# RozDavid/UnScene3D

Measured on AMD Instinct MI355X. Metric: training scenes/sec (Res16UNet34C+Mask3D, 150k voxels), higher is better.
Workload: dtype f32

## Files before the change

### include/usc3d.h

```cpp
#ifndef USC3D_H
#define USC3D_H

#include <stdint.h>

#ifdef __cplusplus
extern "C" {
#endif

typedef void* usc_stream_t;

enum usc_status {
  USC_OK = 0,
  USC_ERR_ARG = -1,
  USC_ERR_LAUNCH = -2,
  USC_ERR_RANGE = -3
};

const char* usc_last_error(void);
int usc_abi_version(void);
const char* usc_build_info(void);
int usc_device_count(void);


int usc_voxel_floor_f64(const double* xyz, int64_t n, double voxel_size,
// ... 550 lines not shown
int usc_adamw_step(float* param, const float* grad, float* exp_avg, float* exp_avg_sq,
                   int64_t n, float lr, float beta1, float beta2, float eps,
                   float weight_decay, int64_t step, usc_stream_t s);

int usc_adamw_step_scaled(float* param, float* grad, float* exp_avg, float* exp_avg_sq, int64_t n,
                          float grad_scale, int32_t write_back_grad,
                          float lr, float beta1, float beta2, float eps, float weight_decay,
                          int64_t step, usc_stream_t s);

int usc_elastic_displace(const void* xyz_in, int32_t is_f64, int64_t n, int32_t row_stride,
                         const float* noise, int32_t dim_x, int32_t dim_y, int32_t dim_z,
                         const double* axis_x, const double* axis_y, const double* axis_z,
                         double magnitude, void* xyz_out, usc_stream_t s);

int usc_affine_rows(void* x, int32_t is_f64, int64_t n, int32_t row_stride,
                    const double* M, const double* t, usc_stream_t s);
int usc_colsum_sequential(const float* x, int64_t n, int32_t row_stride,
                          int32_t cols, float* out, usc_stream_t s);
int usc_color_lut(const float* color, int64_t n, int32_t row_stride,
                  const float* lut, float* out, int32_t out_stride,
                  usc_stream_t s);

int usc_felz_face_normals(const float* vertices, const int32_t* faces,
                          int64_t n_faces, float* face_normals, usc_stream_t s);
int usc_felz_vertex_normals(const float* face_normals, const int64_t* corner_order,
                            const int64_t* vertex_off, int64_t n_vertices,
                            float* normals, usc_stream_t s);
int usc_felz_edge_weights(const float* vertices, const float* colors,
                          const float* normals, const int32_t* faces,
                          int64_t n_faces, int32_t* edge_a, int32_t* edge_b,
                          float* weights, usc_stream_t s);
int usc_felz_merge_host(const int32_t* edge_a, const int32_t* edge_b,
                        const float* weights, int64_t n_edges, int32_t n_vertices,
                        float kthr, int32_t seg_min_verts, int32_t* comps);

int usc_mask_gt_overlap(const uint8_t* masks, int64_t n, int32_t k, int64_t ld,
                        const int32_t* slot, int32_t nslots, int32_t* counts,
                        usc_stream_t s);

int32_t usc_vit_attn_head_dim(void);
int usc_vit_attn_fwd(const float* qkv, int32_t B, int32_t T, int32_t H, float scale,
                     int32_t precision, float* o, usc_stream_t s);

int usc_instance_index(const int64_t* labels, int64_t n, int32_t ld, const int64_t* ids, int32_t u,
                       int32_t* rank, int32_t* count, int32_t* first, usc_stream_t s);
int usc_instance_select(const int64_t* labels, int64_t n, int32_t ld, const int64_t* ids, int32_t u,
                        const int32_t* count, const int32_t* first, const int64_t* filter, int32_t nf,
                        int64_t label_offset, int32_t* slot, int64_t* labels_out, int32_t* n_kept,
                        usc_stream_t s);
int usc_instance_masks(const int32_t* rank, int64_t n, const int32_t* slot, int32_t u, int32_t t,
                       uint8_t* masks, const int64_t* seg, int32_t seg_ld, int64_t n_segments,
                       uint8_t* segment_mask, usc_stream_t s);

int usc_freemask_normalize(const float* feats, int64_t n, int32_t c, float* scale, uint8_t* zero, usc_stream_t s);
int64_t usc_freemask_ws_bytes(int64_t q, int64_t k);
int usc_freemask_rowstats(const float* fq, const float* sq, int64_t q, const float* fk, const float* sk, int64_t k,
                          int32_t c, float* rowmin, float* rowmax, void* ws, int64_t ws_bytes, usc_stream_t s);
int usc_freemask_bits(const float* fq, const float* sq, int64_t q, const float* fk, const float* sk,
                      const uint8_t* zero_k, int64_t k, int32_t c, const float* rowmin, const float* rowmax,
                      float threshold, uint64_t* bits, int32_t* count, float* soft_sum, void* ws, int64_t ws_bytes,
                      usc_stream_t s);
int usc_freemask_soft_rows(const float* fq, const float* sq, int64_t q, const float* fk, const float* sk,
                           const uint8_t* zero_k, int64_t k, int32_t c, const float* rowmin, const float* rowmax,
                           const int32_t* qidx, int32_t m, float* out, usc_stream_t s);
int usc_mask_bits_extent(const uint64_t* bits, int64_t n, int64_t k, const int32_t* coords, int32_t* lo, int32_t* hi,
                         usc_stream_t s);
int64_t usc_mask_bits_nms_ws_bytes(int64_t n);
int usc_mask_bits_nms(const uint64_t* bits, const int32_t* count, int64_t k, const int32_t* order, int32_t n,
                      float nms_thr, uint8_t* keep, void* ws, int64_t ws_bytes, usc_stream_t s);

#define USC_MASK_BITS_MAX_SEGMENTS 8192
int32_t usc_mask_bits_max_segments(void);
int usc_maxpool_down2_i32(const int32_t* in, int64_t n_fine, const int32_t* nbr2, int64_t n_coarse, int32_t* out,
                          usc_stream_t s);
int usc_mask_bits_components(const uint64_t* bits, int64_t n_bits_rows, int32_t n_segments, const int32_t* rows,
                             int32_t n_rows, const int64_t* adj_off, const int32_t* adj, int32_t* label,
                             int32_t* n_comp, usc_stream_t s);
int usc_mask_bits_split(const int32_t* label, int32_t n_rows, int32_t n_segments, const int64_t* row_off,
                        const int32_t* n_comp, const int32_t* weight, const float* soft, int64_t soft_ld,
                        const int32_t* soft_row, uint64_t* out_bits, int32_t* out_src, int32_t* out_root,
                        int32_t* seg_count, int32_t* vox_count, float* soft_sum, usc_stream_t s);
int usc_mask_bits_nms_weighted(const uint64_t* bits, const int32_t* count, const int32_t* weight, int64_t k,
                               const int32_t* order, int32_t n, float nms_thr, uint8_t* keep, void* ws,
                               int64_t ws_bytes, usc_stream_t s);

int64_t usc_softmask_stats_ws_bytes(int64_t n, int32_t k);
int usc_softmask_stats(const float* soft, const float* xyz, int64_t n, int32_t k, float thr, int32_t* count, float* lo,
                       float* hi, void* ws, int64_t ws_bytes, usc_stream_t s);
int usc_softmask_table(const float* soft, int64_t n, int32_t k, float thr, const int32_t* keep, int32_t kk,
                       const float* segments, int32_t* out, usc_stream_t s);
int usc_mesh_vertex_normals(const float* vertices, const int32_t* faces, const int64_t* corner_order,
                            const int64_t* vertex_off, int64_t n_vertices, int64_t n_faces, float* normals,
                            usc_stream_t s);

int usc_mask_columns_to_bits(const uint8_t* masks, int64_t n, int32_t k, uint64_t* bits, int32_t* count,
                             usc_stream_t s);
int usc_mask_bits_gather(const uint64_t* src, int64_t m, const int64_t* ind, int64_t n, int32_t k, uint64_t* dst,
                         int32_t* count, usc_stream_t s);
int usc_mask_bits_count(const uint64_t* bits, int32_t k, int64_t n, int32_t* count, usc_stream_t s);
int32_t usc_selftrain_merge_lds_words(int32_t words);
int usc_selftrain_merge(const uint64_t* st, const int32_t* total, int32_t kp, int64_t n, uint64_t* fg,
                        int32_t max_add, uint64_t* fresh, int32_t* picked, int32_t* n_added, usc_stream_t s);
int usc_mask_bits_to_columns(const uint64_t* bits, const int32_t* rows, int32_t m, int64_t n, float* out, int64_t ld,
                             int32_t col0, usc_stream_t s);
int usc_mask_bits_to_columns_u8(const uint64_t* bits, const int32_t* rows, int32_t m, int64_t n, uint8_t* out,
                                int64_t ld, int32_t col0, usc_stream_t s);
// ... 17 lines not shown
```

### unscene3d_amd/_lib.py

```python
from __future__ import annotations

import ctypes as C
import os

import torch

_HERE = os.path.dirname(os.path.abspath(__file__))
LIB_PATH = os.environ.get("USC3D_LIB") or os.path.join(_HERE, "libusc3d_hip.so")

_p = C.c_void_p
_i32 = C.c_int32
_i64 = C.c_int64
_f64 = C.c_double
_f32 = C.c_float

class KMap(C.Structure):
    _fields_ = [("nbr", _p), ("perm", _p), ("tile_mask", _p), ("pair_in", _p), ("pair_out", _p), ("koff", _p),
                ("n_in", _i64), ("n_out", _i64), ("pair_capacity", _i64), ("K", _i32), ("reserved", _i32)]


class BNDesc(C.Structure):
    _fields_ = [("gamma", _p), ("beta", _p), ("running_mean", _p), ("running_var", _p), ("num_batches_tracked", _p),
                ("eps", _f32), ("momentum", _f32), ("c", _i32), ("training", _i32)]

# ... 152 lines not shown
    "usc_adamw_step_scaled": (C.c_int, [_p, _p, _p, _p, _i64, _f32, _i32, _f32, _f32, _f32, _f32, _f32, _i64, _p]),
    "usc_elastic_displace": (C.c_int, [_p, _i32, _i64, _i32, _p, _i32, _i32, _i32, _p, _p, _p, _f64, _p, _p]),
    "usc_attn_max_queries": (_i32, []),
    "usc_attn_lse_stride": (_i32, [_i32]),
    "usc_attn_ws_bytes": (_i64, [_i32, _i32, _i32, _i32]),
    "usc_attn_fwd": (C.c_int, [_p, _p, _p, _p, _i32, _i32, _i32, _i32, _i32, _p, _p, _p, _i64, _p]),
    "usc_attn_bwd": (C.c_int, [_p, _p, _p, _p, _p, _p, _p, _i32, _i32, _i32, _i32, _i32, _p, _p, _p, _i32, _p, _i64, _p]),
    "usc_lsap_batch": (C.c_int, [_p, _i32, _i32, _i32, _p, _p, _p, _p]),
    "usc_criterion_ws_bytes": (_i64, [_i32, _i32, _i32]),
    "usc_criterion_ws_bytes_q": (_i64, [_i32, _i32, _i32, _i32]),
    "usc_criterion_target_bits": (C.c_int, [_p, _i32, _i32, _i32, _p, _p, _p]),
    "usc_criterion_costs": (C.c_int, [_p, _i32, _i32, _i32, _i32, _i32, _i32, _p, _p, _p, _i64, _i64, _i32, _p, _f32, _f32,
                                      _f32, _p, _p, _p, _p, _p, _p, _p, _i64, _p]),
    "usc_criterion_drop_counts": (C.c_int, [_p, _i32, _i32, _i32, _i32, _i32, _i32, _p, _p, _p, _p, _p]),
    "usc_criterion_losses": (C.c_int, [_p, _p, _p, _p, _p, _p, _p, _i32, _i32, _i32, _i32, _i32, _i32, _p, _p, _p, _p,
                                       _f32, _p, _p]),
    "usc_criterion_table": (C.c_int, [_p, _i32, _i32, _p, _p, _p]),
    "usc_criterion_backward": (C.c_int, [_p, _p, _i32, _i32, _i32, _i32, _i32, _i32, _p, _p, _p, _p, _p, _p, _p, _p, _p,
                                         _p, _p, _i32, _i64, _i64, _p, _p, _p]),
    "usc_self_attn_fwd": (C.c_int, [_p, _p, _p, _i32, _i32, _i32, _i32, _p, _p, _p]),
    "usc_self_attn_bwd": (C.c_int, [_p, _p, _p, _p, _p, _p, _i32, _i32, _i32, _i32, _p, _p, _p, _p]),
    "usc_linear_fwd": (C.c_int, [_p, _p, _p, _i32, _i32, _i32, _p, _p]),
    "usc_linear_bwd": (C.c_int, [_p, _p, _p, _i32, _i32, _i32, _p, _p, _p, _i32, _p]),
    "usc_layernorm_fwd": (C.c_int, [_p, _p, _p, _i64, _i32, _f32, _p, _p, _p, _p]),
    "usc_add_layernorm_fwd": (C.c_int, [_p, _p, _p, _p, _i64, _i32, _f32, _p, _p, _p, _p, _p]),
    "usc_linear_fwd_ex": (C.c_int, [_p, _p, _p, _p, _i32, _i32, _i32, _i32, _p, _p]),
    "usc_linear_fwd_pad": (C.c_int, [_p, _p, _p, _p, _i32, _i32, _i32, _i32, _p, _i32, _p]),
    "usc_linear_fwd_split": (C.c_int, [_p, _p, _p, _p, _i32, _i32, _i32, _i32, _i32, _p, _p]),
    "usc_linear_bwd_ex": (C.c_int, [_p, _p, _p, _p, _p, _i32, _i32, _i32, _p, _p, _p, _p, _i32, _p]),
    "usc_qkv_proj_bwd": (C.c_int, [_p, _p, _p, _p, _i32, _i32, _p, _p, _p, _p, _p, _i32, _p]),
    "usc_linear_bwd_ex2": (C.c_int, [_p, _p, _p, _p, _p, _i32, _i32, _i32, _p, _p, _p, _p, _p, _p, _i32, _p]),
    "usc_linear_heads_max": (_i32, []),
    "usc_linear_heads_dx": (C.c_int, [_p, _p, _i32, _i32, _i32, _i32, _p, _p]),
    "usc_layernorm_bwd_ws_bytes": (_i64, [_i64, _i32]),
    "usc_layernorm_bwd": (C.c_int, [_p, _p, _p, _p, _p, _i64, _i32, _p, _p, _p, _i32, _p, _i64, _p]),
    "usc_layernorm_bwd_ex": (C.c_int, [_p, _p, _p, _p, _p, _i64, _i32, _p, _p, _p, _p, _i32, _p, _i64, _p]),
    "usc_affine_rows": (C.c_int, [_p, _i32, _i64, _i32, _p, _p, _p]),
    "usc_colsum_sequential": (C.c_int, [_p, _i64, _i32, _i32, _p, _p]),
    "usc_col_sum_ws_bytes": (_i64, [_i64, _i32]),
    "usc_col_sum": (C.c_int, [_p, _i64, _i32, _p, _i32, _p, _i64, _p]),
    "usc_color_lut": (C.c_int, [_p, _i64, _i32, _p, _p, _i32, _p]),
    "usc_felz_face_normals": (C.c_int, [_p, _p, _i64, _p, _p]),
    "usc_felz_vertex_normals": (C.c_int, [_p, _p, _p, _i64, _p, _p]),
    "usc_felz_edge_weights": (C.c_int, [_p, _p, _p, _p, _i64, _p, _p, _p, _p]),
    "usc_felz_merge_host": (C.c_int, [_p, _p, _p, _i64, _i32, _f32, _i32, _p]),
    "usc_furthest_point_sampling": (C.c_int, [_p, _i32, _i32, _i32, _p, _p, _p]),
    "usc_fourier_posenc": (C.c_int, [_p, _i64, _p, _p, _p, _i32, _p, _p]),
    "usc_mask_gt_overlap": (C.c_int, [_p, _i64, _i32, _i64, _p, _i32, _p, _p]),
    "usc_vit_attn_head_dim": (_i32, []),
    "usc_vit_attn_fwd": (C.c_int, [_p, _i32, _i32, _i32, _f32, _i32, _p, _p]),
    "usc_instance_index": (C.c_int, [_p, _i64, _i32, _p, _i32, _p, _p, _p, _p]),
    "usc_instance_select": (C.c_int, [_p, _i64, _i32, _p, _i32, _p, _p, _p, _i32, _i64, _p, _p, _p, _p]),
    "usc_instance_masks": (C.c_int, [_p, _i64, _p, _i32, _i32, _p, _p, _i32, _i64, _p, _p]),
    "usc_freemask_normalize": (C.c_int, [_p, _i64, _i32, _p, _p, _p]),
    "usc_freemask_ws_bytes": (_i64, [_i64, _i64]),
    "usc_freemask_rowstats": (C.c_int, [_p, _p, _i64, _p, _p, _i64, _i32, _p, _p, _p, _i64, _p]),
    "usc_freemask_bits": (C.c_int, [_p, _p, _i64, _p, _p, _p, _i64, _i32, _p, _p, _f32, _p, _p, _p, _p, _i64, _p]),
    "usc_freemask_soft_rows": (C.c_int, [_p, _p, _i64, _p, _p, _p, _i64, _i32, _p, _p, _p, _i32, _p, _p]),
    "usc_mask_bits_extent": (C.c_int, [_p, _i64, _i64, _p, _p, _p, _p]),
    "usc_mask_bits_nms_ws_bytes": (_i64, [_i64]),
    "usc_mask_bits_nms": (C.c_int, [_p, _p, _i64, _p, _i32, _f32, _p, _p, _i64, _p]),
    "usc_mask_bits_max_segments": (_i32, []),
    "usc_maxpool_down2_i32": (C.c_int, [_p, _i64, _p, _i64, _p, _p]),
    "usc_mask_bits_components": (C.c_int, [_p, _i64, _i32, _p, _i32, _p, _p, _p, _p, _p]),
    "usc_mask_bits_split": (C.c_int, [_p, _i32, _i32, _p, _p, _p, _p, _i64, _p, _p, _p, _p, _p, _p, _p, _p]),
    "usc_mask_bits_nms_weighted": (C.c_int, [_p, _p, _p, _i64, _p, _i32, _f32, _p, _p, _i64, _p]),
    "usc_softmask_stats_ws_bytes": (_i64, [_i64, _i32]),
    "usc_softmask_stats": (C.c_int, [_p, _p, _i64, _i32, _f32, _p, _p, _p, _p, _i64, _p]),
    "usc_softmask_table": (C.c_int, [_p, _i64, _i32, _f32, _p, _i32, _p, _p, _p]),
    "usc_mesh_vertex_normals": (C.c_int, [_p, _p, _p, _p, _i64, _i64, _p, _p]),
    "usc_mask_columns_to_bits": (C.c_int, [_p, _i64, _i32, _p, _p, _p]),
    "usc_mask_bits_gather": (C.c_int, [_p, _i64, _p, _i64, _i32, _p, _p, _p]),
    "usc_mask_bits_count": (C.c_int, [_p, _i32, _i64, _p, _p]),
    "usc_selftrain_merge_lds_words": (_i32, [_i32]),
    "usc_selftrain_merge": (C.c_int, [_p, _p, _i32, _i64, _p, _i32, _p, _p, _p, _p]),
    "usc_mask_bits_to_columns": (C.c_int, [_p, _p, _i32, _i64, _p, _i64, _i32, _p]),
    "usc_mask_bits_to_columns_u8": (C.c_int, [_p, _p, _i32, _i64, _p, _i64, _i32, _p]),
    "usc_mask_bits_max_segments_wide": (_i32, []),
    "usc_mask_columns_to_segment_bits": (C.c_int, [_p, _i64, _i32, _p, _p, _i32, _p, _p]),
    "usc_mask_bits_components_wide": (C.c_int, [_p, _i64, _i32, _p, _i32, _p, _p, _p, _p, _p, _p]),
    "usc_segment_parts_to_columns": (C.c_int, [_p, _i32, _i32, _p, _p, _i32, _p, _i64, _p, _p]),
}


class LaunchStat(C.Structure):
    _fields_ = [("n_out", _i64), ("cin", _i32), ("cout", _i32), ("K", _i32), ("nb", _i32)]


def _load():
    if not os.path.exists(LIB_PATH):
        raise ImportError(
            f"{LIB_PATH} is missing: build the HIP extension first "
            "(`python -c 'import __graft_entry__ as g; g.build()'`). "
            "unscene3d_amd has no CPU fallback."
        )
    lib = C.CDLL(LIB_PATH)
    for name, (res, args) in SIGNATURES.items():
        fn = getattr(lib, name)
        fn.restype = res
        fn.argtypes = args
    return lib


lib = _load()
if lib.usc_step_size() != C.sizeof(Step):
    raise ImportError(f"unscene3d_amd._lib.Step ({C.sizeof(Step)} bytes) does not mirror usc_step "
# ... 19 lines not shown
```

### unscene3d_amd/csrc/targets.hip

```cpp
#include "common.h"

namespace usc {

constexpr int kTgtBlock = 256;
constexpr int kTgtWindow = 2048;
constexpr int kTgtWaveRows = 256;
constexpr int kTgtRowsPerBlock = 8;

__global__ void instance_index_init_kernel(int32_t u, int32_t* __restrict__ count, int32_t* __restrict__ first) {
  for (int32_t i = blockIdx.x * blockDim.x + threadIdx.x; i < u; i += gridDim.x * blockDim.x) {
    count[i] = 0;
    first[i] = INT32_MAX;
  }
}

__device__ inline int32_t find_rank(const int64_t* __restrict__ ids, int32_t u, int64_t v) {
  int32_t lo = 0, hi = u;
  while (lo < hi) {
    const int32_t mid = (lo + hi) >> 1;
    if (ids[mid] < v) lo = mid + 1; else hi = mid;
  }
  return (lo < u && ids[lo] == v) ? lo : -1;
}

// ... 87 lines not shown
  const int64_t base = ((int64_t)blockIdx.x * (kTgtBlock / 64) + wave) * kTgtWaveRows;
  if (base >= n) return;
  const int len = (int)min((int64_t)kTgtWaveRows, n - base);

  int32_t sl[4];
#pragma unroll
  for (int k = 0; k < 4; ++k) {
    const int64_t r = base + 64 * k + lane;
    sl[k] = -1;
    if (r < n) {
      const int32_t q = rank[r];
      if ((uint32_t)q < (uint32_t)u) {
        const int32_t t = slot[q];
        if ((uint32_t)t < (uint32_t)t_total) sl[k] = t;
      }
    }
  }
  if (segment_mask != nullptr && blockIdx.y == 0) {
#pragma unroll
    for (int k = 0; k < 4; ++k) {
      if (sl[k] >= 0) {
        const int64_t sg = seg[(base + 64 * k + lane) * seg_ld];
        if ((uint64_t)sg < (uint64_t)s) segment_mask[(int64_t)sl[k] * s + sg] = 1;
      }
    }
  }

  const int t0 = blockIdx.y * kTgtRowsPerBlock;
  const int t1 = min(t_total, t0 + kTgtRowsPerBlock);
  for (int t = t0; t < t1; ++t) {
    const uint64_t b0 = __ballot(sl[0] == t), b1 = __ballot(sl[1] == t);
    const uint64_t b2 = __ballot(sl[2] == t), b3 = __ballot(sl[3] == t);
    uint8_t* row = masks + (int64_t)t * n + base;
    const int m = (int)((uintptr_t)row & 3);
    const int j_lo = m ? 1 : 0;
    const int j_hi = (len + m) >> 2;
    if (lane >= j_lo && lane < j_hi) {
      const int i0 = 4 * lane - m;
      const int q = i0 >> 6, o = i0 & 63;
      const uint64_t cur = q == 0 ? b0 : q == 1 ? b1 : q == 2 ? b2 : b3;
      const uint64_t nxt = q == 0 ? b1 : q == 1 ? b2 : q == 2 ? b3 : 0;
      uint32_t bits = (uint32_t)(cur >> o);
      if (o > 60) bits |= (uint32_t)(nxt << (64 - o));
      const uint32_t word = (bits & 1u) | ((bits & 2u) << 7) | ((bits & 4u) << 14) | ((bits & 8u) << 21);
      *reinterpret_cast<uint32_t*>(row + i0) = word;
    }
    const int head_n = min(max(4 * j_lo - m, 0), len);
    if (lane < head_n) row[lane] = (uint8_t)ballot_bit(b0, b1, b2, b3, lane);
    const int tail = max(4 * j_hi - m, head_n) + lane;
    if (tail < len) row[tail] = (uint8_t)ballot_bit(b0, b1, b2, b3, tail);
  }
}

}

using namespace usc;

extern "C" {

int usc_instance_index(const int64_t* labels, int64_t n, int32_t ld, const int64_t* ids, int32_t u, int32_t* rank,
                       int32_t* count, int32_t* first, usc_stream_t s) {
  USC_REQUIRE(n >= 0 && n < INT32_MAX, "usc_instance_index: n out of range [0, 2^31-2]");
  USC_REQUIRE(ld >= 2, "usc_instance_index: ld < 2 (the instance id is column 1)");
  USC_REQUIRE(u >= 0 && u <= 65535 * kTgtWindow, "usc_instance_index: u out of range");
  USC_REQUIRE(u == 0 || (ids && count && first), "usc_instance_index: null pointer");
  USC_REQUIRE(n == 0 || (labels && rank), "usc_instance_index: null pointer");
  USC_REQUIRE(n == 0 || u > 0, "usc_instance_index: rows without ids");
  hipStream_t st = as_stream(s);
  if (u == 0) return USC_OK;
  hipLaunchKernelGGL(instance_index_init_kernel, dim3(stream_grid(u, kTgtBlock)), dim3(kTgtBlock), 0, st, u, count,
                     first);
  USC_CHECK_LAUNCH("usc_instance_index");
  if (n == 0) return USC_OK;
  const dim3 grid(stream_grid(n, kTgtBlock), (unsigned)ceil_div(u, kTgtWindow));
  hipLaunchKernelGGL(instance_index_kernel, grid, dim3(kTgtBlock), 0, st, labels, n, ld, ids, u, rank, count, first);
  USC_CHECK_LAUNCH("usc_instance_index");
  return USC_OK;
}

int usc_instance_select(const int64_t* labels, int64_t n, int32_t ld, const int64_t* ids, int32_t u,
                        const int32_t* count, const int32_t* first, const int64_t* filter, int32_t nf,
                        int64_t label_offset, int32_t* slot, int64_t* labels_out, int32_t* n_kept, usc_stream_t s) {
  USC_REQUIRE(n >= 0 && n < INT32_MAX, "usc_instance_select: n out of range [0, 2^31-2]");
  USC_REQUIRE(ld >= 1, "usc_instance_select: ld < 1");
  USC_REQUIRE(u >= 0, "usc_instance_select: u < 0");
  USC_REQUIRE(nf >= 0 && (nf == 0 || filter), "usc_instance_select: bad filter list");
  USC_REQUIRE(n_kept, "usc_instance_select: null n_kept");
  USC_REQUIRE(u == 0 || (labels && ids && count && first && slot && labels_out), "usc_instance_select: null pointer");
  hipLaunchKernelGGL(instance_select_kernel, dim3(1), dim3(kTgtBlock), 0, as_stream(s), labels, ld, ids, u, count,
                     first, filter, nf, label_offset, slot, labels_out, n_kept);
  USC_CHECK_LAUNCH("usc_instance_select");
  return USC_OK;
}

int usc_instance_masks(const int32_t* rank, int64_t n, const int32_t* slot, int32_t u, int32_t t, uint8_t* masks,
                       const int64_t* seg, int32_t seg_ld, int64_t n_segments, uint8_t* segment_mask,
                       usc_stream_t s) {
  USC_REQUIRE(n >= 0 && n < INT32_MAX, "usc_instance_masks: n out of range [0, 2^31-2]");
  USC_REQUIRE(u >= 0, "usc_instance_masks: u < 0");
  USC_REQUIRE(t >= 0 && t <= u && t <= 65535 * kTgtRowsPerBlock, "usc_instance_masks: t out of range [0, u]");
  USC_REQUIRE(n_segments >= 0, "usc_instance_masks: n_segments < 0");
  if (t == 0 || n == 0) return USC_OK;
  USC_REQUIRE(rank && slot && masks, "usc_instance_masks: null pointer");
  if (n_segments == 0) segment_mask = nullptr;
  USC_REQUIRE(segment_mask == nullptr || (seg && seg_ld >= 1), "usc_instance_masks: segment_mask without segment ids");
  const dim3 grid((unsigned)ceil_div(n, (kTgtBlock / 64) * kTgtWaveRows), (unsigned)ceil_div(t, kTgtRowsPerBlock));
  hipLaunchKernelGGL(instance_masks_kernel, grid, dim3(kTgtBlock), 0, as_stream(s), rank, n, slot, u, t, masks, seg,
                     seg_ld, n_segments, segment_mask);
  USC_CHECK_LAUNCH("usc_instance_masks");
  return USC_OK;
}
// ... 3 lines not shown
```

### unscene3d_amd/datasets/utils.py

```python
from __future__ import annotations

import numpy as np
import torch

from .. import MinkowskiEngine as ME
from .. import ops


def _dev(x, dev, dtype):
    t = x if isinstance(x, torch.Tensor) else torch.as_tensor(np.asarray(x))
    return t.to(device=dev, dtype=dtype).contiguous()


class NoGpu:

    def __init__(self, coordinates, features, original_labels=None, inverse_maps=None, full_res_coords=None,
                 target_full=None, original_colors=None, original_normals=None, original_coordinates=None, idx=None,
                 segment_connectivity=None):
        self.coordinates, self.features = coordinates, features
        self.original_labels, self.inverse_maps, self.full_res_coords = original_labels, inverse_maps, full_res_coords
        self.target_full, self.original_colors, self.original_normals = target_full, original_colors, original_normals
        self.original_coordinates, self.idx, self.segment_connectivity = original_coordinates, idx, segment_connectivity


def get_instance_freemasks(list_freemasks, list_segments=None):
    target = []
    for b, table in enumerate(list_freemasks):
        colsT = (table[:, 1:-1] != 0).T.contiguous()
        keep = torch.nonzero(colsT.any(1)).reshape(-1)
        if keep.numel() == 0:
            return []
        masks = colsT[keep]
        entry = {"labels": torch.ones(keep.numel(), dtype=torch.int64, device=table.device), "masks": masks}
        if list_segments:
            S = list_segments[b].shape[0]
            tt, rr = torch.nonzero(masks, as_tuple=True)
            vals = table[rr]
            sm = torch.zeros((keep.numel(), S), dtype=torch.bool, device=table.device)
            sm[tt[:, None].expand_as(vals).reshape(-1), vals.reshape(-1)] = True
            entry["segment_mask"] = sm
        target.append(entry)
    return target


def freemask_voxelize(batch, ignore_label, voxel_size, mode, ignore_class_threshold, device="cuda",
                      spatial_sort=False):
    dev = torch.device(device)
    coords_l, feats_l, tables, inverse_maps = [], [], [], []
    full_res_coords, original_freemasks, colors, normals, raw_coords, idx, seg_conn = [], [], [], [], [], [], []
    for sample in batch:
        full_res_coords.append(sample[0])
        original_freemasks.append(sample[2])
        colors.append(sample[4])
        normals.append(sample[5])
        raw_coords.append(sample[6])
        idx.append(sample[7])
        seg_conn.append(sample[8])
        xyz = _dev(sample[0], dev, torch.float64)
        c3, unique_map, inverse_map = ME.utils.sparse_quantize(xyz, quantization_size=voxel_size, return_index=True,
                                                               return_inverse=True, device=str(dev))
        if spatial_sort:
            c4 = torch.cat([torch.zeros((c3.shape[0], 1), dtype=torch.int32, device=dev), c3], 1).contiguous()
            order = ops.spatial_order(c4, shift=int(spatial_sort) if spatial_sort is not True else 3)
            rank = torch.empty_like(order)
            rank[order] = torch.arange(order.shape[0], device=dev)
            c3, unique_map, inverse_map = c3[order], unique_map[order], rank[inverse_map]
        inverse_maps.append(inverse_map)
        coords_l.append(c3.int())
        feats_l.append(_dev(sample[1], dev, torch.float32)[unique_map])
        if len(sample[2]) > 0:
            tables.append(_dev(sample[2], dev, torch.int64)[unique_map])

    if tables:
        width = max(t.shape[1] for t in tables)
        tables = [torch.cat([t[:, :-1], t.new_zeros(t.shape[0], width - t.shape[1]), t[:, -1:]], dim=1) for t in tables]
        coordinates, features, _ = ME.utils.sparse_collate(coords_l, feats_l, tables)
    else:
        coordinates, features = ME.utils.sparse_collate(coords_l, feats_l)

    target, target_full = [], []
    if tables:
        segment2label, n_segments = [], []
        for t in tables:
            seg = t[:, -1]
            uniq, inv = torch.unique(seg, return_inverse=True)
            n_segments.append(int(uniq.shape[0]))
            first = torch.full((uniq.shape[0],), seg.shape[0], dtype=torch.long, device=dev)
            first.scatter_reduce_(0, inv, torch.arange(seg.shape[0], device=dev), reduce="amin")
            t[:, -1] = inv
            segment2label.append(t[first][:, :-1])
        target = get_instance_freemasks(tables, list_segments=segment2label)
        for i in range(len(target)):
            target[i]["point2segment"] = tables[i][:, -1].contiguous()
            target[i]["num_segments"] = torch.tensor(n_segments[i])
        full = [m if isinstance(m, torch.Tensor) else torch.as_tensor(np.asarray(m)) for m in original_freemasks]
        target_full = get_instance_freemasks(full)
        for i in range(len(target_full)):
            target_full[i]["point2segment"] = full[i][:, -1].long()
    else:
        coordinates, features = [], []
    return (NoGpu(coordinates, features, original_freemasks, inverse_maps, full_res_coords, target_full, colors,
                  normals, raw_coords, idx, seg_conn), target, [sample[3] for sample in batch])


class FreeMaskVoxelizeCollate:
    def __init__(self, ignore_label=255, voxel_size=1, mode="test", small_crops=False, very_small_crops=False,
                 batch_instance=False, probing=False, task="instance_segmentation", ignore_class_threshold=100,
                 filter_out_classes=(), label_offset=0, num_queries=None, device="cuda", spatial_sort=False):
        assert task in ["instance_segmentation"], "task not known"
        if small_crops or very_small_crops:
            raise NotImplementedError("crop collates are outside the accelerated path (SURVEY.md §2.1)")
        self.ignore_label, self.voxel_size, self.mode = ignore_label, voxel_size, mode
        self.ignore_class_threshold, self.device, self.spatial_sort = ignore_class_threshold, device, spatial_sort

    def __call__(self, batch):
        return freemask_voxelize(batch, self.ignore_label, self.voxel_size, self.mode, self.ignore_class_threshold,
                                 device=self.device, spatial_sort=self.spatial_sort)


def get_instance_masks(list_labels, task, list_segments=None, ignore_class_threshold=100, filter_out_classes=(),
                       label_offset=0):
    if task == "semantic_segmentation":
        raise NotImplementedError("task='semantic_segmentation' targets are outside the accelerated path (SURVEY.md §2.1)")
    target = []
# ... 116 lines not shown
```

### unscene3d_amd/ops.py

```python
from __future__ import annotations

from dataclasses import dataclass

import ctypes
import os
import weakref

import torch

from . import profiler as _prof
from ._lib import check, lib, require_device


def _stream():
    return torch._C._cuda_getCurrentRawStream(torch._C._cuda_getDevice())


def _chk(t: torch.Tensor, dtype, name: str):
    if not isinstance(t, torch.Tensor):
        raise RuntimeError(f"{name} must be a torch.Tensor")
    if not t.is_cuda:
        raise RuntimeError(f"{name} must be a HIP (cuda) tensor — unscene3d_amd has no CPU path")
    if t.dtype != dtype:
        raise RuntimeError(f"{name} must be {dtype}, got {t.dtype}")
# ... 983 lines not shown
                            _ptr(d2), _ptr(ws), ws.numel(), _stream()), "usc_knn1_grid")
    return d2.sqrt(), idx


def mask_gt_overlap(masks: torch.Tensor, slot: torch.Tensor, nslots: int) -> torch.Tensor:
    require_device()
    if not isinstance(masks, torch.Tensor) or masks.dim() != 2 or not masks.is_cuda:
        raise RuntimeError("masks must be a 2-D HIP (cuda) tensor")
    if masks.dtype == torch.bool:
        masks = masks.view(torch.uint8)
    if masks.dtype != torch.uint8:
        raise RuntimeError(f"masks must be bool or uint8, got {masks.dtype}")
    n, k = masks.shape
    if n > 0 and (masks.stride(1) != 1 or masks.stride(0) < k):
        masks = masks.contiguous()
    ld = masks.stride(0) if n > 0 else k
    _chk(slot, torch.int32, "slot")
    if slot.shape != (n,):
        raise RuntimeError(f"slot must be [{n}], got {list(slot.shape)}")
    counts = torch.empty((k + 1, int(nslots)), dtype=torch.int32, device=masks.device)
    check(lib.usc_mask_gt_overlap(_ptr(masks), n, k, ld, _ptr(slot), int(nslots), _ptr(counts), _stream()),
          "usc_mask_gt_overlap")
    return counts


def instance_targets(labels: torch.Tensor, num_segments=None, filter_out_classes=(), label_offset: int = 0, alloc=None):
    require_device()
    _chk(labels, torch.int64, "labels")
    if labels.dim() != 2 or labels.shape[1] < (2 if num_segments is None else 3):
        raise RuntimeError("labels must be [N, >= 2] (with segments: [N, >= 3])")
    dev = labels.device
    if alloc is None:
        def alloc(shape, dtype, zero):
            return (torch.zeros if zero else torch.empty)(shape, dtype=dtype, device=dev)
    n, ld = labels.shape
    ids = torch.unique(labels[:, 1]).contiguous()
    u = int(ids.shape[0])
    rank, count, first = alloc((n,), torch.int32, False), alloc((u,), torch.int32, False), alloc((u,), torch.int32, False)
    slot, lab, kept = alloc((u,), torch.int32, False), alloc((u,), torch.int64, False), alloc((1,), torch.int32, False)
    flt = torch.tensor([int(c) for c in filter_out_classes], dtype=torch.int64, device=dev)
    st = _stream()
    check(lib.usc_instance_index(_ptr(labels), n, ld, _ptr(ids), u, _ptr(rank), _ptr(count), _ptr(first), st),
          "usc_instance_index")
    check(lib.usc_instance_select(_ptr(labels), n, ld, _ptr(ids), u, _ptr(count), _ptr(first), _ptr(flt),
                                  int(flt.shape[0]), int(label_offset), _ptr(slot), _ptr(lab), _ptr(kept), st),
          "usc_instance_select")
    t = int(kept.item())
    masks = alloc((t, n), torch.uint8, False)
    seg_mask = None if num_segments is None else alloc((t, int(num_segments)), torch.uint8, True)
    check(lib.usc_instance_masks(_ptr(rank), n, _ptr(slot), u, t, _ptr(masks), _ptr(labels[:, 2:]) if seg_mask is not None
                                 else None, ld, 0 if seg_mask is None else int(num_segments), _ptr(seg_mask), st),
          "usc_instance_masks")
    return lab[:t], masks.view(torch.bool), None if seg_mask is None else seg_mask.view(torch.bool)


VIT_ATTN_PRECISIONS = {"f32": 0, "bf16": 1}


def vit_attention(qkv: torch.Tensor, B: int, T: int, H: int, scale: float, precision: str = "f32") -> torch.Tensor:
    require_device()
    _chk(qkv, torch.float32, "qkv")
    if precision not in VIT_ATTN_PRECISIONS:
        raise RuntimeError(f"precision must be 'f32' or 'bf16', got {precision!r}")
    d = lib.usc_vit_attn_head_dim()
    if qkv.numel() != B * T * 3 * H * d:
        raise RuntimeError(f"qkv must hold [B={B}, T={T}, 3, H={H}, {d}] values, got {list(qkv.shape)}")
    o = torch.empty((B, T, H * d), dtype=torch.float32, device=qkv.device)
    check(lib.usc_vit_attn_fwd(_ptr(qkv), B, T, H, float(scale), VIT_ATTN_PRECISIONS[precision], _ptr(o), _stream()),
          "usc_vit_attn_fwd")
    return o


def cc_eps(xyz: torch.Tensor, eps: float, max_rounds: int = 256) -> torch.Tensor:
    require_device()
    _chk(xyz, torch.float32, "xyz")
    n = xyz.shape[0]
    dev = xyz.device
    la = torch.empty(n, dtype=torch.int32, device=dev)
    lb = torch.empty(n, dtype=torch.int32, device=dev)
    changed = torch.zeros(1, dtype=torch.int32, device=dev)
    check(lib.usc_cc_eps_init(_ptr(la), n, _stream()), "usc_cc_eps_init")
    for _ in range(max_rounds):
        check(lib.usc_cc_eps_step(_ptr(xyz), n, float(eps), _ptr(la), _ptr(lb), _ptr(changed), _stream()),
              "usc_cc_eps_step")
        la, lb = lb, la
        if int(changed.item()) == 0:
            break
    else:
        raise RuntimeError("cc_eps: label propagation did not converge")
    labels = torch.empty(n, dtype=torch.int64, device=dev)
    check(lib.usc_cc_eps_finish(_ptr(la), n, _ptr(lb), _ptr(labels), _stream()), "usc_cc_eps_finish")
    return labels


DBSCAN_OFF = -2
DBSCAN_MAX_CELLS_PER_AXIS = 1 << 20


def dbscan_masks(xyz: torch.Tensor, masks: torch.Tensor, eps: float, min_samples: int = 1):
    require_device()
    _chk(xyz, torch.float32, "xyz")
    _chk(masks, torch.float32, "masks")
    if xyz.dim() != 2 or xyz.shape[1] != 3 or masks.dim() != 2 or masks.shape[0] != xyz.shape[0]:
        raise RuntimeError(f"dbscan_masks: xyz must be [N,3] and masks [N,Q], got {list(xyz.shape)}, {list(masks.shape)}")
    eps32 = ctypes.c_float(float(eps)).value
    if not (eps32 > 0.0) or eps32 == float("inf"):
# ... 740 lines not shown
```

Before: 46.84.

## Build freemask training targets natively with hash-based segment indexing on GPU

Adds native HIP kernels that scan the per-scene label table once, find which mask columns are non-empty, build a hash table of segment ids, rank them, and emit masks, point2segment and segment masks directly. This replaces the torch-op path (gather, unique, pad, scatter_reduce, per-target mask building) in freemask_voxelize and is enabled by default through an environment flag. The new path needs one pinned-memory readback per table to learn the target and segment counts. The rank kernel is quadratic in the number of segments and the collate path now skips the padded-table concatenation.

```diff
diff --git a/include/usc3d.h b/include/usc3d.h
--- a/include/usc3d.h
+++ b/include/usc3d.h
@@ -626,6 +626,17 @@
                        uint8_t* masks, const int64_t* seg, int32_t seg_ld, int64_t n_segments,
                        uint8_t* segment_mask, usc_stream_t s);
 
+int64_t usc_freemask_targets_ws_bytes(int64_t n, int32_t W, int32_t with_segments);
+int usc_freemask_targets_index(const void* src, int32_t src_i64, int32_t W, const int64_t* rows,
+                               int64_t n_src, int64_t n, int32_t with_segments, void* ws,
+                               int64_t ws_bytes, int64_t* out_table, int32_t Wp, int64_t* host_counts,
+                               usc_stream_t s);
+int usc_freemask_targets_emit(const void* src, int32_t src_i64, int32_t W, const int64_t* rows,
+                              int64_t n_src, int64_t n, int32_t with_segments, void* ws,
+                              int64_t ws_bytes, int32_t T, int64_t S, uint8_t* masks, int64_t* labels,
+                              int64_t* point2segment, uint8_t* segment_mask, int64_t* out_table,
+                              int32_t Wp, int64_t* segment2label, usc_stream_t s);
+
 int usc_freemask_normalize(const float* feats, int64_t n, int32_t c, float* scale, uint8_t* zero, usc_stream_t s);
 int64_t usc_freemask_ws_bytes(int64_t q, int64_t k);
 int usc_freemask_rowstats(const float* fq, const float* sq, int64_t q, const float* fk, const float* sk, int64_t k,
diff --git a/unscene3d_amd/_lib.py b/unscene3d_amd/_lib.py
--- a/unscene3d_amd/_lib.py
+++ b/unscene3d_amd/_lib.py
@@ -228,6 +228,10 @@
     "usc_instance_index": (C.c_int, [_p, _i64, _i32, _p, _i32, _p, _p, _p, _p]),
     "usc_instance_select": (C.c_int, [_p, _i64, _i32, _p, _i32, _p, _p, _p, _i32, _i64, _p, _p, _p, _p]),
     "usc_instance_masks": (C.c_int, [_p, _i64, _p, _i32, _i32, _p, _p, _i32, _i64, _p, _p]),
+    "usc_freemask_targets_ws_bytes": (_i64, [_i64, _i32, _i32]),
+    "usc_freemask_targets_index": (C.c_int, [_p, _i32, _i32, _p, _i64, _i64, _i32, _p, _i64, _p, _i32, _p, _p]),
+    "usc_freemask_targets_emit": (C.c_int, [_p, _i32, _i32, _p, _i64, _i64, _i32, _p, _i64, _i32, _i64, _p, _p, _p, _p,
+                                            _p, _i32, _p, _p]),
     "usc_freemask_normalize": (C.c_int, [_p, _i64, _i32, _p, _p, _p]),
     "usc_freemask_ws_bytes": (_i64, [_i64, _i64]),
     "usc_freemask_rowstats": (C.c_int, [_p, _p, _i64, _p, _p, _i64, _i32, _p, _p, _p, _i64, _p]),
diff --git a/unscene3d_amd/csrc/targets.hip b/unscene3d_amd/csrc/targets.hip
--- a/unscene3d_amd/csrc/targets.hip
+++ b/unscene3d_amd/csrc/targets.hip
@@ -163,11 +163,344 @@
   }
 }
 
+constexpr int kFmBlock = 256;
+constexpr int kFmMaxCols = 1024;
+constexpr int kFmTile = 1024;
+constexpr int64_t kFmEmpty = INT64_MIN;
+
+struct FmWs {
+  int64_t* counts;
+  int32_t* colflag;
+  int32_t* col_of_t;
+  int64_t* hkeys;
+  int32_t* hidx;
+  int64_t* distinct;
+  int32_t* rslot;
+  int32_t* rank;
+  int32_t* first;
+  int64_t cap, bytes;
+};
+
+static int64_t fm_cap(int64_t n) {
+  int64_t cap = 1024;
+  while (cap < 2 * n) cap <<= 1;
+  return cap;
+}
+
+static FmWs fm_carve(void* ws, int64_t n, int32_t K, bool with_seg) {
+  FmWs w{};
+  char* p = (char*)ws;
+  int64_t o = 0;
+  auto take = [&](int64_t bytes) { char* q = p + o; o += align_up(bytes, 16); return q; };
+  w.counts = (int64_t*)take(32);
+  w.colflag = (int32_t*)take((int64_t)K * 4);
+  w.col_of_t = (int32_t*)take((int64_t)K * 4);
+  if (with_seg) {
+    w.cap = fm_cap(n);
+    w.hkeys = (int64_t*)take(w.cap * 8);
+    w.hidx = (int32_t*)take(w.cap * 4);
+    w.distinct = (int64_t*)take(n * 8);
+    w.rslot = (int32_t*)take(n * 4);
+    w.rank = (int32_t*)take(n * 4);
+    w.first = (int32_t*)take(n * 4);
+  }
+  w.bytes = o;
+  return w;
+}
+
+__global__ void fm_init_kernel(int64_t* __restrict__ counts, int32_t* __restrict__ colflag, int32_t K,
+                               int64_t* __restrict__ hkeys, int64_t cap) {
+  const int64_t i0 = (int64_t)blockIdx.x * blockDim.x + threadIdx.x;
+  if (i0 < 4) counts[i0] = 0;
+  if (i0 < K) colflag[i0] = 0;
+  for (int64_t i = i0; i < cap; i += (int64_t)gridDim.x * blockDim.x) hkeys[i] = kFmEmpty;
+}
+
+template <typename TS>
+__global__ __launch_bounds__(kFmBlock) void fm_scan_kernel(const TS* __restrict__ src, int32_t W,
+                                                           const int64_t* __restrict__ rows, int64_t n_src, int64_t n,
+                                                           int64_t* __restrict__ hkeys, int32_t* __restrict__ hidx,
+                                                           int64_t cap, int64_t* __restrict__ distinct,
+                                                           int32_t* __restrict__ rslot, int32_t* __restrict__ colflag,
+                                                           int64_t* __restrict__ counts, int64_t* __restrict__ out_table,
+                                                           int32_t Wp) {
+  __shared__ int32_t sflag[kFmMaxCols];
+  const int K = W - 2;
+  for (int i = threadIdx.x; i < K; i += kFmBlock) sflag[i] = 0;
+  __syncthreads();
+  for (int64_t r = (int64_t)blockIdx.x * kFmBlock + threadIdx.x; r < n; r += (int64_t)gridDim.x * kFmBlock) {
+    const int64_t q = rows ? rows[r] : r;
+    if ((uint64_t)q >= (uint64_t)n_src) {
+      counts[2] = 1;
+      if (rslot) rslot[r] = -1;
+      continue;
+    }
+    const TS* __restrict__ p = src + q * W;
+    for (int c = 0; c < K; ++c)
+      if (p[1 + c] != 0 && !sflag[c]) sflag[c] = 1;
+    const int64_t sg = (int64_t)p[W - 1];
+    if (rslot) {
+      int32_t mine = -1;
+      if (sg == kFmEmpty) {
+        counts[2] = 1;
+      } else {
+        uint64_t slot = hash_key((uint64_t)sg) & (uint64_t)(cap - 1);
+        for (;;) {
+          if (__atomic_load_n(&hkeys[slot], __ATOMIC_RELAXED) == sg) break;
+          const unsigned long long prev = atomicCAS((unsigned long long*)&hkeys[slot], (unsigned long long)kFmEmpty,
+                                                    (unsigned long long)sg);
+          if (prev == (unsigned long long)kFmEmpty) {
+            const int64_t di = (int64_t)atomicAdd((unsigned long long*)&counts[1], 1ull);
+            distinct[di] = sg;
+            hidx[slot] = (int32_t)di;
+            break;
+          }
+          if (prev == (unsigned long long)sg) break;
+          slot = (slot + 1) & (uint64_t)(cap - 1);
+        }
+        mine = (int32_t)slot;
+      }
+      rslot[r] = mine;
+    }
+    if (out_table) {
+      int64_t* __restrict__ o = out_table + r * Wp;
+      for (int c = 0; c < W - 1; ++c) o[c] = (int64_t)p[c];
+      for (int c = W - 1; c < Wp - 1; ++c) o[c] = 0;
+      o[Wp - 1] = sg;
+    }
+  }
+  __syncthreads();
+  for (int i = threadIdx.x; i < K; i += kFmBlock)
+    if (sflag[i]) colflag[i] = 1;
+}
+
+__global__ void fm_count_kernel(const int32_t* __restrict__ colflag, int32_t K, int32_t* __restrict__ col_of_t,
+                                int64_t* __restrict__ counts) {
+  if (threadIdx.x != 0 || blockIdx.x != 0) return;
+  int32_t t = 0;
+  for (int32_t c = 0; c < K; ++c)
+    if (colflag[c]) col_of_t[t++] = c;
+  counts[0] = t;
+}
+
+__global__ __launch_bounds__(kFmBlock) void fm_rank_kernel(const int64_t* __restrict__ distinct, int64_t S,
+                                                           int32_t* __restrict__ rank, int32_t* __restrict__ first,
+                                                           int64_t* __restrict__ labels, int32_t T) {
+  __shared__ int64_t tile[kFmTile];
+  const int64_t i = (int64_t)blockIdx.x * kFmBlock + threadIdx.x;
+  const int64_t v = i < S ? distinct[i] : 0;
+  int32_t below = 0;
+  for (int64_t j0 = 0; j0 < S; j0 += kFmTile) {
+    const int m = (int)min((int64_t)kFmTile, S - j0);
+    __syncthreads();
+    for (int k = threadIdx.x; k < m; k += kFmBlock) tile[k] = distinct[j0 + k];
+    __syncthreads();
+    for (int k = 0; k < m; ++k) below += tile[k] < v ? 1 : 0;
+  }
+  if (i < S) {
+    rank[i] = below;
+    first[i] = INT32_MAX;
+  }
+  if (i < T) labels[i] = 1;
+}
+
+__device__ inline void fm_mark(uint8_t* __restrict__ row, int64_t S, int64_t v) {
+  if (v < 0) v += S;
+  if ((uint64_t)v < (uint64_t)S) row[v] = 1;
+}
+
+template <typename TS>
+__global__ __launch_bounds__(kFmBlock) void fm_rows_kernel(const TS* __restrict__ src, int32_t W,
+                                                           const int64_t* __restrict__ rows, int64_t n_src, int64_t n,
+                                                           int32_t Wp, int32_t T, int64_t S,
+                                                           const int32_t* __restrict__ col_of_t,
+                                                           const int32_t* __restrict__ rslot,
+                                                           const int32_t* __restrict__ hidx,
+                                                           const int32_t* __restrict__ rank, int32_t* __restrict__ first,
+                                                           int32_t want_first, uint8_t* __restrict__ masks,
+                                                           int64_t* __restrict__ p2s, uint8_t* __restrict__ segmask,
+                                                           int64_t* __restrict__ out_table) {
+  __shared__ int32_t scol[kFmMaxCols];
+  for (int i = threadIdx.x; i < T; i += kFmBlock) scol[i] = col_of_t[i];
+  __syncthreads();
+  const int lane = threadIdx.x & 63;
+  const int K = W - 2;
+  for (int64_t base = (int64_t)blockIdx.x * kFmBlock; base < n; base += (int64_t)gridDim.x * kFmBlock) {
+    const int64_t r = base + threadIdx.x;
+    bool valid = r < n;
+    int64_t q = 0;
+    if (valid) {
+      q = rows ? rows[r] : r;
+      if ((uint64_t)q >= (uint64_t)n_src) { valid = false; q = 0; }
+    }
+    const TS* __restrict__ p = src + q * W;
+    int64_t rk = -1;
+    if (valid && rslot) {
+      const int32_t slot = rslot[r];
+      if (slot >= 0) {
+        rk = rank[hidx[slot]];
+        p2s[r] = rk;
+        if (out_table) out_table[r * Wp + Wp - 1] = rk;
+        if (want_first && rk < S) atomicMin(&first[rk], (int32_t)r);
+      }
+    }
+    bool has0 = false, has1 = false, odd = false;
+    int64_t lab = 0;
+    if (valid && segmask) {
+      lab = (int64_t)p[0];
+      has0 = Wp > W || lab == 0 || rk == 0;
+      has1 = lab == 1 || rk == 1;
+      for (int c = 0; c < K; ++c) {
+        const int64_t v = (int64_t)p[1 + c];
+        has0 = has0 || v == 0;
+        has1 = has1 || v == 1;
+        odd = odd || (v != 0 && v != 1);
+      }
+    }
+    for (int t = 0; t < T; ++t) {
+      const bool bit = valid && p[1 + scol[t]] != 0;
+      if (r < n) masks[(int64_t)t * n + r] = bit ? 1 : 0;
+      if (segmask) {
+        uint8_t* __restrict__ row = segmask + (int64_t)t * S;
+        const uint64_t b0 = __ballot(bit && has0), b1 = __ballot(bit && has1);
+        if (b0 && S > 0 && lane == __ffsll((unsigned long long)b0) - 1) row[0] = 1;
+        if (b1 && S > 1 && lane == __ffsll((unsigned long long)b1) - 1) row[1] = 1;
+        if (bit) {
+          if (rk > 1 && rk < S) row[rk] = 1;
+          if (lab != 0 && lab != 1) fm_mark(row, S, lab);
+          if (odd)
+            for (int c = 0; c < K; ++c) {
+              const int64_t v = (int64_t)p[1 + c];
+              if (v != 0 && v != 1) fm_mark(row, S, v);
+            }
+        }
+      }
+    }
+  }
+}
+
+template <typename TS>
+__global__ void fm_seg2label_kernel(const TS* __restrict__ src, int32_t W, const int64_t* __restrict__ rows,
+                                    int64_t n_src, int64_t n, int32_t Wp, int64_t S,
+                                    const int32_t* __restrict__ first, int64_t* __restrict__ out) {
+  const int64_t total = S * (Wp - 1);
+  for (int64_t e = (int64_t)blockIdx.x * blockDim.x + threadIdx.x; e < total; e += (int64_t)gridDim.x * blockDim.x) {
+    const int64_t sgm = e / (Wp - 1);
+    const int c = (int)(e - sgm * (Wp - 1));
+    const int64_t fr = first[sgm];
+    const int64_t q = fr >= n ? -1 : rows ? rows[fr] : fr;
+    out[e] = (c < W - 1 && (uint64_t)q < (uint64_t)n_src) ? (int64_t)src[q * W + c] : 0;
+  }
+}
+
+static thread_local int64_t* g_fm_pinned = nullptr;
+
 }
 
 using namespace usc;
 
 extern "C" {
+
+int64_t usc_freemask_targets_ws_bytes(int64_t n, int32_t W, int32_t with_segments) {
+  if (n < 0 || W < 2) return 0;
+  return fm_carve(nullptr, n, W - 2, with_segments != 0).bytes;
+}
+
+int usc_freemask_targets_index(const void* src, int32_t src_i64, int32_t W, const int64_t* rows, int64_t n_src,
+                               int64_t n, int32_t with_segments, void* ws, int64_t ws_bytes, int64_t* out_table,
+                               int32_t Wp, int64_t* host_counts, usc_stream_t s) {
+  USC_REQUIRE(n >= 0 && n < INT32_MAX && n_src >= 0, "usc_freemask_targets_index: n out of range [0, 2^31-2]");
+  USC_REQUIRE(W >= 2 && W - 2 <= kFmMaxCols, "usc_freemask_targets_index: table width %d outside [2, %d]", W,
+              kFmMaxCols + 2);
+  USC_REQUIRE(Wp >= W, "usc_freemask_targets_index: padded width below the table's");
+  USC_REQUIRE(ws && host_counts, "usc_freemask_targets_index: null pointer");
+  USC_REQUIRE(n == 0 || src, "usc_freemask_targets_index: null table");
+  USC_REQUIRE(ws_bytes >= usc_freemask_targets_ws_bytes(n, W, with_segments),
+              "usc_freemask_targets_index: workspace too small");
+  USC_REQUIRE(out_table == nullptr || with_segments, "usc_freemask_targets_index: the gathered table needs segments");
+  hipStream_t st = as_stream(s);
+  const int32_t K = W - 2;
+  const FmWs w = fm_carve(ws, n, K, with_segments != 0);
+  if (g_fm_pinned == nullptr) {
+    hipError_t e = hipHostMalloc((void**)&g_fm_pinned, 64, hipHostMallocDefault);
+    if (e != hipSuccess) {
+      g_fm_pinned = nullptr;
+      set_error("usc_freemask_targets_index: hipHostMalloc: %s", hipGetErrorString(e));
+      return USC_ERR_LAUNCH;
+    }
+  }
+  const int64_t init_items = w.cap > kFmMaxCols ? w.cap : kFmMaxCols;
+  hipLaunchKernelGGL(fm_init_kernel, dim3(stream_grid(init_items, kFmBlock)), dim3(kFmBlock), 0, st, w.counts,
+                     w.colflag, K, w.hkeys, w.cap);
+  if (n > 0) {
+    const dim3 grid(stream_grid(n, kFmBlock));
+    if (src_i64)
+      hipLaunchKernelGGL(fm_scan_kernel<int64_t>, grid, dim3(kFmBlock), 0, st, (const int64_t*)src, W, rows, n_src, n,
+                         w.hkeys, w.hidx, w.cap, w.distinct, w.rslot, w.colflag, w.counts, out_table, Wp);
+    else
+      hipLaunchKernelGGL(fm_scan_kernel<int32_t>, grid, dim3(kFmBlock), 0, st, (const int32_t*)src, W, rows, n_src, n,
+                         w.hkeys, w.hidx, w.cap, w.distinct, w.rslot, w.colflag, w.counts, out_table, Wp);
+  }
+  hipLaunchKernelGGL(fm_count_kernel, dim3(1), dim3(64), 0, st, w.colflag, K, w.col_of_t, w.counts);
+  USC_CHECK_LAUNCH("usc_freemask_targets_index");
+  hipError_t e = hipMemcpyAsync(g_fm_pinned, w.counts, 32, hipMemcpyDeviceToHost, st);
+  if (e == hipSuccess) e = hipStreamSynchronize(st);
+  if (e != hipSuccess) {
+    set_error("usc_freemask_targets_index: read-back failed: %s", hipGetErrorString(e));
+    return USC_ERR_LAUNCH;
+  }
+  host_counts[0] = g_fm_pinned[0];
+  host_counts[1] = g_fm_pinned[1];
+  host_counts[2] = g_fm_pinned[2];
+  USC_REQUIRE(g_fm_pinned[2] == 0, "usc_freemask_targets_index: a row index outside the table, or segment id INT64_MIN");
+  return USC_OK;
+}
+
+int usc_freemask_targets_emit(const void* src, int32_t src_i64, int32_t W, const int64_t* rows, int64_t n_src,
+                              int64_t n, int32_t with_segments, void* ws, int64_t ws_bytes, int32_t T, int64_t S,
+                              uint8_t* masks, int64_t* labels, int64_t* point2segment, uint8_t* segment_mask,
+                              int64_t* out_table, int32_t Wp, int64_t* segment2label, usc_stream_t s) {
+  USC_REQUIRE(n >= 0 && n < INT32_MAX && n_src >= 0, "usc_freemask_targets_emit: n out of range [0, 2^31-2]");
+  USC_REQUIRE(W >= 2 && W - 2 <= kFmMaxCols && Wp >= W, "usc_freemask_targets_emit: bad table width");
+  USC_REQUIRE(T >= 0 && T <= W - 2 && S >= 0 && S <= n, "usc_freemask_targets_emit: T / S out of range");
+  USC_REQUIRE(ws && ws_bytes >= usc_freemask_targets_ws_bytes(n, W, with_segments),
+              "usc_freemask_targets_emit: workspace too small");
+  USC_REQUIRE(with_segments || (!point2segment && !segment_mask && !out_table && !segment2label),
+              "usc_freemask_targets_emit: segment outputs without segments");
+  USC_REQUIRE(!with_segments || point2segment || n == 0, "usc_freemask_targets_emit: null point2segment");
+  USC_REQUIRE(T == 0 || labels, "usc_freemask_targets_emit: null labels");
+  USC_REQUIRE(T == 0 || n == 0 || masks, "usc_freemask_targets_emit: null masks");
+  hipStream_t st = as_stream(s);
+  const FmWs w = fm_carve(ws, n, W - 2, with_segments != 0);
+  if (segment_mask && T > 0 && S > 0) (void)hipMemsetAsync(segment_mask, 0, (size_t)T * (size_t)S, st);
+  const int64_t rank_items = S > T ? S : T;
+  if (rank_items > 0)
+    hipLaunchKernelGGL(fm_rank_kernel, dim3((unsigned)ceil_div(rank_items, kFmBlock)), dim3(kFmBlock), 0, st,
+                       w.distinct, with_segments ? S : 0, w.rank, w.first, labels, T);
+  if (n > 0) {
+    USC_REQUIRE(src, "usc_freemask_targets_emit: null table");
+    const dim3 grid(stream_grid(n, kFmBlock));
+    if (src_i64)
+      hipLaunchKernelGGL(fm_rows_kernel<int64_t>, grid, dim3(kFmBlock), 0, st, (const int64_t*)src, W, rows, n_src, n,
+                         Wp, T, S, w.col_of_t, w.rslot, w.hidx, w.rank, w.first, segment2label ? 1 : 0, masks,
+                         point2segment, S > 0 ? segment_mask : nullptr, out_table);
+    else
+      hipLaunchKernelGGL(fm_rows_kernel<int32_t>, grid, dim3(kFmBlock), 0, st, (const int32_t*)src, W, rows, n_src, n,
+                         Wp, T, S, w.col_of_t, w.rslot, w.hidx, w.rank, w.first, segment2label ? 1 : 0, masks,
+                         point2segment, S > 0 ? segment_mask : nullptr, out_table);
+    if (segment2label && S > 0 && Wp > 1) {
+      const dim3 g2(stream_grid(S * (Wp - 1), kFmBlock));
+      if (src_i64)
+        hipLaunchKernelGGL(fm_seg2label_kernel<int64_t>, g2, dim3(kFmBlock), 0, st, (const int64_t*)src, W, rows, n_src,
+                           n, Wp, S, w.first, segment2label);
+      else
+        hipLaunchKernelGGL(fm_seg2label_kernel<int32_t>, g2, dim3(kFmBlock), 0, st, (const int32_t*)src, W, rows, n_src,
+                           n, Wp, S, w.first, segment2label);
+    }
+  }
+  USC_CHECK_LAUNCH("usc_freemask_targets_emit");
+  return USC_OK;
+}
 
 int usc_instance_index(const int64_t* labels, int64_t n, int32_t ld, const int64_t* ids, int32_t u, int32_t* rank,
                        int32_t* count, int32_t* first, usc_stream_t s) {
diff --git a/unscene3d_amd/datasets/utils.py b/unscene3d_amd/datasets/utils.py
--- a/unscene3d_amd/datasets/utils.py
+++ b/unscene3d_amd/datasets/utils.py
@@ -1,10 +1,14 @@
 from __future__ import annotations
+
+import os
 
 import numpy as np
 import torch
 
 from .. import MinkowskiEngine as ME
 from .. import ops
+
+NATIVE_TARGETS = os.environ.get("USC3D_NATIVE_TARGETS", "1") == "1"
 
 
 def _dev(x, dev, dtype):
@@ -43,9 +47,38 @@
     return target
 
 
+def _native_table(x, dev):
+    t = x if isinstance(x, torch.Tensor) else torch.as_tensor(np.asarray(x))
+    if t.dtype not in (torch.int32, torch.int64):
+        t = t.to(torch.int64)
+    return t.to(dev).contiguous()
+
+
+def _native_freemask_targets(tables, width):
+    target = []
+    for src, rows in tables:
+        r = ops.freemask_targets(src, rows, segments=True, width=width)
+        if r["n_targets"] == 0:
+            return []
+        target.append({"labels": r["labels"], "masks": r["masks"], "segment_mask": r["segment_mask"],
+                       "point2segment": r["point2segment"], "num_segments": torch.tensor(r["n_segments"])})
+    return target
+
+
+def _native_full_targets(full):
+    target_full = []
+    for t in full:
+        r = ops.freemask_targets(t, None, segments=False)
+        if r["n_targets"] == 0:
+            return []
+        target_full.append({"labels": r["labels"], "masks": r["masks"]})
+    return target_full
+
+
 def freemask_voxelize(batch, ignore_label, voxel_size, mode, ignore_class_threshold, device="cuda",
                       spatial_sort=False):
     dev = torch.device(device)
+    native = NATIVE_TARGETS
     coords_l, feats_l, tables, inverse_maps = [], [], [], []
     full_res_coords, original_freemasks, colors, normals, raw_coords, idx, seg_conn = [], [], [], [], [], [], []
     for sample in batch:
@@ -69,7 +102,21 @@
         coords_l.append(c3.int())
         feats_l.append(_dev(sample[1], dev, torch.float32)[unique_map])
         if len(sample[2]) > 0:
-            tables.append(_dev(sample[2], dev, torch.int64)[unique_map])
+            tables.append((_native_table(sample[2], dev), unique_map.contiguous()) if native
+                          else _dev(sample[2], dev, torch.int64)[unique_map])
+
+    if tables and native:
+        coordinates, features = ME.utils.sparse_collate(coords_l, feats_l)
+        target = _native_freemask_targets(tables, max(t.shape[1] for t, _ in tables))
+        full = [m if isinstance(m, torch.Tensor) else torch.as_tensor(np.asarray(m)) for m in original_freemasks]
+        if all(m.is_cuda and m.dim() == 2 and m.dtype in (torch.int32, torch.int64) for m in full):
+            target_full = _native_full_targets([m.contiguous() for m in full])
+        else:
+            target_full = get_instance_freemasks(full)
+        for i in range(len(target_full)):
+            target_full[i]["point2segment"] = full[i][:, -1].long()
+        return (NoGpu(coordinates, features, original_freemasks, inverse_maps, full_res_coords, target_full, colors,
+                      normals, raw_coords, idx, seg_conn), target, [sample[3] for sample in batch])
 
     if tables:
         width = max(t.shape[1] for t in tables)
diff --git a/unscene3d_amd/ops.py b/unscene3d_amd/ops.py
--- a/unscene3d_amd/ops.py
+++ b/unscene3d_amd/ops.py
@@ -1059,6 +1059,55 @@
                                  else None, ld, 0 if seg_mask is None else int(num_segments), _ptr(seg_mask), st),
           "usc_instance_masks")
     return lab[:t], masks.view(torch.bool), None if seg_mask is None else seg_mask.view(torch.bool)
+
+
+def freemask_targets(table: torch.Tensor, rows=None, segments: bool = True, width=None, want_table: bool = False,
+                     want_segment2label: bool = False, alloc=None):
+    require_device()
+    if not isinstance(table, torch.Tensor) or not table.is_cuda or table.dim() != 2 or not table.is_contiguous():
+        raise RuntimeError("table must be a contiguous 2-D HIP tensor")
+    if table.dtype not in (torch.int32, torch.int64):
+        raise RuntimeError(f"table must be int32 or int64, got {table.dtype}")
+    n_src, W = table.shape
+    if W < 2:
+        raise RuntimeError("table must be [N, >= 2]: label | mask columns | segment id")
+    if rows is not None:
+        _chk(rows, torch.int64, "rows")
+    n = n_src if rows is None else int(rows.shape[0])
+    Wp = W if width is None else int(width)
+    dev = table.device
+    if alloc is None:
+        def alloc(shape, dtype):
+            return torch.empty(shape, dtype=dtype, device=dev)
+    seg = 1 if segments else 0
+    i64 = 1 if table.dtype == torch.int64 else 0
+    ws = alloc((max(int(lib.usc_freemask_targets_ws_bytes(n, W, seg)), 16),), torch.uint8)
+    out_table = alloc((n, Wp), torch.int64) if (segments and want_table) else None
+    counts = (ctypes.c_int64 * 3)()
+    st = _stream()
+    check(lib.usc_freemask_targets_index(_ptr(table), i64, W, _ptr(rows), n_src, n, seg, _ptr(ws), ws.numel(),
+                                         _ptr(out_table), Wp, counts, st), "usc_freemask_targets_index")
+    T, S = int(counts[0]), int(counts[1])
+    out = {"n_targets": T, "n_segments": S if segments else None}
+    masks = alloc((T, n), torch.uint8) if T else None
+    labels = alloc((T,), torch.int64) if T else None
+    p2s = alloc((n,), torch.int64) if segments else None
+    seg_mask = alloc((T, S), torch.uint8) if (segments and T) else None
+    s2l = alloc((S, Wp - 1), torch.int64) if (segments and want_segment2label) else None
+    check(lib.usc_freemask_targets_emit(_ptr(table), i64, W, _ptr(rows), n_src, n, seg, _ptr(ws), ws.numel(), T, S,
+                                        _ptr(masks), _ptr(labels), _ptr(p2s), _ptr(seg_mask), _ptr(out_table), Wp,
+                                        _ptr(s2l), st), "usc_freemask_targets_emit")
+    if T:
+        out["masks"], out["labels"] = masks.view(torch.bool), labels
+        if seg_mask is not None:
+            out["segment_mask"] = seg_mask.view(torch.bool)
+    if segments:
+        out["point2segment"] = p2s
+        if out_table is not None:
+            out["table"] = out_table
+        if s2l is not None:
+            out["segment2label"] = s2l
+    return out
 
 
 VIT_ATTN_PRECISIONS = {"f32": 0, "bf16": 1}
```

Measured after the change: 47.26, median of 6. No clear change (+0.9%).
